# greatscottgadgets/libbtbb

Hardware: AMD Instinct MI355X
Metric: Gbit/s raw bitstream scanned (LAP_ANY, err<=2) (higher is better)
Workload: dtype u64; 1 GPU; promiscuous LAP_ANY scan, 4 GiB packed single-channel synthetic bitstream per GPU, max_ac_errors=2, sync word every 4096 symbols; symbols_per_gpu=34359738305, hits_per_gpu=6402406, parallelism=time-sharded x1 (btbbx_shard_plan: slices + 63-symbol halo), no collectives

## Files before the change

### libbtbb_amd/csrc/context.cpp

```cpp
#include <stdarg.h>
#include <stdio.h>
#include <stdlib.h>
#include <string.h>
#include <mutex>
#include <shared_mutex>
#include <vector>
#include "common.h"

#define NO_DEVICE_SLOT BTBBX_MAX_DEVICES
static Ctx g_ctx[BTBBX_MAX_DEVICES + 1];
static std::mutex g_init_lock;
static std::shared_mutex g_tables_lock;

void ctx_scan_snapshot(ScanTables *tables, int *table_errors)
{
	std::shared_lock<std::shared_mutex> g(g_tables_lock);
	const Ctx &c = ctx();
	*tables = c.scan;
	*table_errors = c.table_errors;
}
static int g_table_errors = 0;
static thread_local char g_err[512] = "";

static int current_device()
// ... 527 lines not shown
	return BTBBX_OK;
}

static int init_current_device(int max_ac_errors)
{
	const int dev = current_device();
	if (dev == NO_DEVICE_SLOT) {
		int d = -1;
		(void)hipGetDevice(&d);
		set_error("btbbx_init: HIP device ordinal %d is not below BTBBX_MAX_DEVICES = %d (or hipGetDevice failed)", d,
			  BTBBX_MAX_DEVICES);
		return BTBBX_E_ARG;
	}
	Ctx &c = g_ctx[dev];
	if (g_table_errors == 0 && max_ac_errors > 0)
		g_table_errors = max_ac_errors;
	if (!c.ready) {
		int n = 0;
		hipError_t e = hipGetDeviceCount(&n);
		if (e != hipSuccess || n <= 0) {
			set_error("btbbx_init: no HIP device available (%s) -- this library has no CPU path",
				  e == hipSuccess ? "device count 0" : hipGetErrorString(e));
			return BTBBX_E_NODEVICE;
		}
		c.device = dev;
		hipDeviceProp_t prop;
		HIP_TRY(hipGetDeviceProperties(&prop, dev));
		c.num_cus = prop.multiProcessorCount > 0 ? prop.multiProcessorCount : 256;
		int rc = chain_upload(host_tables());
		if (rc)
			return rc;
		rc = upload_tables(g_table_errors);
		if (rc)
			return rc;
		c.ready = true;
		return BTBBX_OK;
	}
	if (c.table_errors != g_table_errors)
		return upload_tables(g_table_errors);
	return BTBBX_OK;
}

extern "C" int btbbx_init(int max_ac_errors)
{
	if (max_ac_errors < 0 || max_ac_errors > 5) {
		set_error("btbbx_init: max_ac_errors out of range");
		return BTBBX_E_ARG;
	}
	std::lock_guard<std::mutex> g(g_init_lock);
	return init_current_device(max_ac_errors);
}

extern "C" int btbbx_init_devices(const int *devices, int n_devices, int max_ac_errors)
{
	if (max_ac_errors < 0 || max_ac_errors > 5 || n_devices < 0 || (n_devices && !devices)) {
		set_error("btbbx_init_devices: bad argument");
		return BTBBX_E_ARG;
	}
	const int have = btbbx_device_count();
	int home = 0;
	if (have <= 0 || hipGetDevice(&home) != hipSuccess) {
		set_error("btbbx_init_devices: no HIP device available -- this library has no CPU path");
		return BTBBX_E_NODEVICE;
	}
	std::lock_guard<std::mutex> g(g_init_lock);
	int rc = BTBBX_OK;
	for (int i = 0; i < n_devices && !rc; i++) {
		if (devices[i] < 0 || devices[i] >= have || devices[i] >= BTBBX_MAX_DEVICES) {
			set_error("btbbx_init_devices: device %d does not exist (%d visible)", devices[i], have);
			rc = BTBBX_E_ARG;
			break;
		}
		if (hipSetDevice(devices[i]) != hipSuccess)
			rc = hip_fail(hipGetLastError(), "hipSetDevice");
		else
			rc = init_current_device(max_ac_errors);
	}
	(void)hipSetDevice(home);
	return rc;
}

void hop_pool_release();
void sort_scratch_release();

extern "C" void btbbx_shutdown(void)
{
	std::lock_guard<std::mutex> g(g_init_lock);
	int home = 0;
	(void)hipGetDevice(&home);
	hop_pool_release();
	sort_scratch_release();
	for (int d = 0; d < BTBBX_MAX_DEVICES; d++) {
		Ctx &c = g_ctx[d];
		std::vector<CallBufs *> mine;
		{
			std::lock_guard<std::mutex> p(g_pool_lock);
			mine.swap(g_pool[d]);
		}
		if (!c.ready && mine.empty())
			continue;
		(void)hipSetDevice(d);
		for (CallBufs *b : mine)
			bufs_free(b);
		if (c.d_tab_block) (void)hipFree(c.d_tab_block);
		if (c.d_hslots) (void)hipFree(c.d_hslots);
		if (c.d_bitmap2) (void)hipFree(c.d_bitmap2);
		if (c.d_retired_tab) (void)hipFree(c.d_retired_tab);
		if (c.d_retired_hslots) (void)hipFree(c.d_retired_hslots);
		if (c.d_retired_bitmap2) (void)hipFree(c.d_retired_bitmap2);
		c = Ctx();
	}
	g_table_errors = 0;
	(void)hipSetDevice(home);
}


extern "C" void *btbbx_malloc(size_t bytes)
{
	void *p = nullptr;
	hipError_t e = hipMalloc(&p, bytes);
	if (e != hipSuccess) {
		hip_fail(e, "hipMalloc");
		return nullptr;
	}
	return p;
}

extern "C" void btbbx_free(void *p)
{
	if (p)
		(void)hipFree(p);
}

extern "C" int btbbx_memcpy_h2d(void *dst, const void *src, size_t bytes)
{
	HIP_TRY(hipMemcpy(dst, src, bytes, hipMemcpyHostToDevice));
	return BTBBX_OK;
}

extern "C" int btbbx_memcpy_d2h(void *dst, const void *src, size_t bytes)
{
	HIP_TRY(hipMemcpy(dst, src, bytes, hipMemcpyDeviceToHost));
	return BTBBX_OK;
}

extern "C" int btbbx_memset(void *p, int value, size_t bytes)
{
	HIP_TRY(hipMemset(p, value, bytes));
	return BTBBX_OK;
}

extern "C" int btbbx_sync(void *hip_stream)
{
	HIP_TRY(hipStreamSynchronize((hipStream_t)hip_stream));
	return BTBBX_OK;
}
```

### libbtbb_amd/csrc/packet.hip

```cpp
#include <stdlib.h>
#include <string.h>
#include <atomic>
#include <type_traits>
#include "packet_launch.h"
#include "packet_core.h"

static uint32_t host_crc_byte(uint32_t crc, uint32_t byte)
{
	uint32_t x = (crc ^ byte) & 0xff;
	x ^= (x << 4) & 0xff;
	return ((crc >> 8) ^ (x << 8) ^ (x << 3) ^ (x >> 4)) & 0xffff;
}

int chain_upload(const HostTables &t)
{
	{
		int seen[16] = {0};
		for (int clk = 0; clk < 64; clk++) {
			uint32_t v = 0;
			for (int j = 0; j < 4; j++)
				v |= (uint32_t)t.whiten[(t.whiten_idx[clk] + 3 + j) % 127] << j;
			seen[v]++;
		}
		for (int v = 0; v < 16; v++)
			if (seen[v] != 4) {
				set_error("btbbx_init: internal: the type-field whitening is not four clocks per value");
				return BTBBX_E_ARG;
			}
	}
	{
		static ChainLds img;
		memset(&img, 0, sizeof(img));
		for (int i = 0; i < 128; i++)
			for (int j = 0; j < 32; j++)
				img.wh32[i] |= (uint32_t)t.whiten[((i < 127 ? i : 0) + j) % 127] << j;
		for (int i = 0; i < 256; i++) {
			uint32_t c = host_crc_byte(0, (uint32_t)i);
			img.crc[i] = (uint16_t)c;
			for (int k = 0; k < 3; k++) {
				c = host_crc_byte(c, 0);
				img.crc_z[k][i] = (uint16_t)c;
			}
		}
		for (int i = 0; i < 1024; i++) {
			uint32_t par = 0;
			for (int bit = 0; bit < 10; bit++)
				if ((i >> bit) & 1)
					par ^= t.fec23_par[bit];
			img.par23[i] = (uint8_t)par;
		}
		memcpy(img.fix23, t.fec23_fix, 32);
		for (int i = 0; i < 32; i++)
			img.fixm23[i] = t.fec23_fix[i] == -2 ? 0x8000u : t.fec23_fix[i] >= 0 ? (uint16_t)(1u << t.fec23_fix[i]) : 0u;
		memcpy(img.whiten_idx, t.whiten_idx, 64);
		for (int h = 0; h < 2; h++)
			for (int i = 0; i < 256; i++) {
				uint32_t c = (uint32_t)i << (8 * h);
				for (int k = 0; k < 32; k++)
					c = host_crc_byte(c, 0);
				img.adv32[h][i] = (uint16_t)c;
			}
		HIP_TRY(hipMemcpyToSymbol(HIP_SYMBOL(g_chain_lds_image), &img, sizeof(img)));
	}
	{
		static uint16_t lin[LIN_MAXLEN * 16];
		memset(lin, 0, sizeof(lin));
		for (int bit = 0; bit < 8; bit++) {
			uint32_t crc = 1u << (8 + bit);
			for (int L = 0; L < LIN_MAXLEN; L++) {
				lin[L * 16 + bit] = (uint16_t)crc;
				crc = host_crc_byte(crc, 0);
			}
		}
		uint32_t taps = 0;
		for (uint32_t m = 1; m < 128 && !taps; m++) {
			bool ok = true;
			for (int k = 0; k < 127 && ok; k++) {
				uint32_t x = 0;
				for (int j = 0; j < 7; j++)
					if ((m >> j) & 1)
						x ^= t.whiten[(k + j) % 127];
				ok = x == t.whiten[(k + 7) % 127];
			}
			if (ok)
				taps = m;
// ... 94 lines not shown
	if (d_count)
		n_packets = min(n_packets, *d_count);
	uint32_t pkt = blockIdx.x * GATHER_PACKETS + threadIdx.x / BTBBX_PKT_WORDS;
	uint32_t i = threadIdx.x % BTBBX_PKT_WORDS;
	if (pkt >= n_packets || threadIdx.x >= GATHER_PACKETS * BTBBX_PKT_WORDS)
		return;
	const btbbx_hit h = hits[pkt];
	const uint64_t *base = words + (uint64_t)h.stream * pitch_words;
	uint64_t total_bits = n_words * 64;
	uint64_t avail = h.offset < total_bits ? total_bits - h.offset : 0;
	uint32_t len = avail < max_length ? (uint32_t)avail : max_length;
	if (len > BTBBX_MAX_SYMBOLS)
		len = BTBBX_MAX_SYMBOLS;
	uint64_t bit = h.offset + 64ULL * i;
	uint64_t j = bit >> 6;
	uint32_t sh = (uint32_t)(bit & 63);
	uint64_t lo = j < n_words ? base[j] : 0, hi = (j + 1) < n_words ? base[j + 1] : 0;
	uint64_t v = sh ? (lo >> sh) | (hi << (64 - sh)) : lo;
	uint32_t first = 64 * i;
	if (first >= len)
		v = 0;
	else if (len - first < 64)
		v &= (1ULL << (len - first)) - 1;
	packets[(uint64_t)pkt * BTBBX_PKT_WORDS + i] = v;
	if (i == 0)
		lengths[pkt] = len;
}

__global__ __launch_bounds__(256) void header_flags_kernel(const uint64_t *packets, const uint32_t *lengths, uint32_t n_packets,
							    uint8_t *present, const uint32_t *d_count)
{
	const uint32_t i = blockIdx.x * 256 + threadIdx.x;
	if (i >= n_packets || (d_count && i >= *d_count))
		return;
	PState s;
	s.w = packets + (uint64_t)i * BTBBX_PKT_WORDS;
	s.length = (int)lengths[i];
	present[i] = (uint8_t)do_header_present(s);
}

int launch_trials_state(const uint8_t *d_sym, const btbbx_pkt_in *d_in, const btbbx_pkt_out *d_out, void *d_state,
			btbbx_trial *d_trials, hipStream_t stream)
{
	int rc = ctx_require();
	if (rc)
		return rc;
	hipLaunchKernelGGL(trials_state_kernel, dim3(64), dim3(64), 0, stream, d_sym, d_in, d_out, (TrialState *)d_state, d_trials);
	HIP_TRY(hipGetLastError());
	return BTBBX_OK;
}

int launch_trials_merge(const void *d_state, const btbbx_pkt_in *d_in, btbbx_pkt_out *d_out, uint8_t *d_pay,
			const TrialPlan *plan, hipStream_t stream)
{
	hipLaunchKernelGGL(trials_merge_kernel, dim3(1), dim3(64), 0, stream, (const TrialState *)d_state, d_in, d_out, d_pay,
			   *plan);
	HIP_TRY(hipGetLastError());
	return BTBBX_OK;
}

size_t trials_state_bytes() { return 64 * sizeof(TrialState); }

int launch_gather(const uint64_t *d_words, uint64_t n_words, uint64_t pitch_words, const btbbx_hit *d_hits, uint32_t n_packets,
		  const uint32_t *d_count, uint32_t max_length, uint64_t *d_packets, uint32_t *d_lengths, hipStream_t hip_stream)
{
	int rc = ctx_require();
	if (rc)
		return rc;
	if (!n_packets)
		return BTBBX_OK;
	hipLaunchKernelGGL(gather_kernel, dim3((n_packets + GATHER_PACKETS - 1) / GATHER_PACKETS), dim3(256), 0,
			   hip_stream, d_words, n_words, pitch_words, d_hits, n_packets, max_length, d_packets, d_lengths, d_count);
	HIP_TRY(hipGetLastError());
	return BTBBX_OK;
}

extern "C" int btbbx_gather_packets_device(const uint64_t *d_words, uint64_t n_words, uint64_t pitch_words,
					   const btbbx_hit *d_hits, uint32_t n_packets, uint32_t max_length,
					   uint64_t *d_packets, uint32_t *d_lengths, void *hip_stream)
{
	return launch_gather(d_words, n_words, pitch_words, d_hits, n_packets, nullptr, max_length, d_packets, d_lengths, (hipStream_t)hip_stream);
}

extern "C" int btbbx_trials_device(const uint64_t *d_packets, const btbbx_pkt_in *d_in, uint32_t n_packets,
				   btbbx_trial *d_trials, void *hip_stream)
{
	return launch_trials(d_packets, d_in, n_packets, nullptr, d_trials, (hipStream_t)hip_stream);
}

int launch_trials(const uint64_t *d_packets, const btbbx_pkt_in *d_in, uint32_t n_packets, const uint32_t *d_count,
		  btbbx_trial *d_trials, hipStream_t hip_stream)
{
	int rc = ctx_require();
	if (rc)
		return rc;
	if (!n_packets)
		return BTBBX_OK;
	if (n_packets <= 256) {
		hipLaunchKernelGGL(trials_wide_kernel, dim3(n_packets * 64), dim3(64), 0, (hipStream_t)hip_stream,
				   d_packets, d_in, n_packets, d_trials, d_count);
	} else {
		const uint32_t batches = (n_packets + TL_PACKETS - 1) / TL_PACKETS;
		const uint32_t resident = (uint32_t)ctx().num_cus * TL_WGS_PER_CU;
		hipLaunchKernelGGL(trials_linear_kernel, dim3(batches < resident ? batches : resident), dim3(TL_THREADS), 0,
				   (hipStream_t)hip_stream, d_packets, d_in, n_packets, d_trials, d_count);
	}
#ifdef TL_PROFILE
	if (n_packets > 256) {
		unsigned long long prof[16], tot = 0;
		(void)hipDeviceSynchronize();
		(void)hipMemcpyFromSymbol(prof, HIP_SYMBOL(g_tl_prof), sizeof(prof));
		for (int k = 0; k < 16; k++) tot += prof[k];
		fprintf(stderr, "trials profile:");
		for (int k = 0; k < 10; k++) fprintf(stderr, " %d:%.1f%%", k, 100.0 * (double)prof[k] / (double)(tot ? tot : 1));
		fprintf(stderr, "\n");
		static unsigned long long z[16];
		(void)hipMemcpyToSymbol(HIP_SYMBOL(g_tl_prof), z, sizeof(z));
	}
#endif
	HIP_TRY(hipGetLastError());
	return BTBBX_OK;
}

extern "C" int btbbx_uap_table_device(const uint64_t *d_packets, const btbbx_pkt_in *d_in, uint32_t n_packets,
				      uint16_t *d_table, void *hip_stream)
{
	int rc = ctx_require();
	if (rc)
		return rc;
	if (!n_packets)
		return BTBBX_OK;
	if ((uintptr_t)d_table & 15) {
		set_error("btbbx_uap_table_device: table must be 16-byte aligned");
		return BTBBX_E_ARG;
	}
	hipLaunchKernelGGL(uap_table_kernel, dim3((n_packets + 255) / 256), dim3(256), 0, (hipStream_t)hip_stream,
			   d_packets, d_in, n_packets, (uint4 *)d_table);
	HIP_TRY(hipGetLastError());
	return BTBBX_OK;
}

int launch_header_flags(const uint64_t *d_packets, const uint32_t *d_lengths, uint32_t n_packets, const uint32_t *d_count,
			uint8_t *d_present, hipStream_t stream)
{
	if (!n_packets)
		return BTBBX_OK;
	hipLaunchKernelGGL(header_flags_kernel, dim3((n_packets + 255) / 256), dim3(256), 0, stream, d_packets, d_lengths, n_packets, d_present, d_count);
	HIP_TRY(hipGetLastError());
	return BTBBX_OK;
}

int launch_decode_bytes(const uint8_t *d_sym, uint8_t *d_pay, const btbbx_pkt_in *d_in, btbbx_pkt_out *d_out,
			uint32_t mode, bool with_payload, hipStream_t stream)
{
	int rc = ctx_require();
	if (rc)
		return rc;
	hipLaunchKernelGGL(decode_bytes_kernel, dim3(1), dim3(64), 0, stream, d_sym, d_pay, d_in, d_out, mode,
			   with_payload ? 1 : 0);
	HIP_TRY(hipGetLastError());
	return BTBBX_OK;
}

int launch_decode(const uint64_t *d_packets, const btbbx_pkt_in *d_in, uint32_t n_packets,
		  btbbx_pkt_out *d_out, uint32_t mode, const TrialPlan *plan, hipStream_t stream)
{
	int rc = ctx_require();
	if (rc)
		return rc;
	if (!n_packets)
		return BTBBX_OK;
	TrialPlan p = {0, 0, 0};
	if (plan)
		p = *plan;
	if (mode & DEC_TRIALS) {
		if (mode != DEC_TRIALS || n_packets != 1) {
			set_error("decode: trial replay is a one-packet mode");
			return BTBBX_E_ARG;
		}
		hipLaunchKernelGGL(replay_kernel, dim3(1), dim3(64), 0, stream, d_packets, d_in, d_out, p);
		HIP_TRY(hipGetLastError());
		return BTBBX_OK;
	}
	hipLaunchKernelGGL(decode_kernel, dim3((n_packets + 63) / 64), dim3(64), 0, stream,
			   d_packets, d_in, n_packets, d_out, mode);
	HIP_TRY(hipGetLastError());
	return BTBBX_OK;
}

extern "C" int btbbx_decode_device(const uint64_t *d_packets, const btbbx_pkt_in *d_in, uint32_t n_packets,
// ... 134 lines not shown
```

### libbtbb_amd/csrc/packet_trials.h

```cpp
#pragma once


__device__ __forceinline__ uint32_t lds_now(const uint32_t *p)
{
	return *(volatile __attribute__((address_space(3))) const uint32_t *)p;
}

#define TL_THREADS 512
#define TL_PACKETS (TL_THREADS / 16)
#define TL_WGS_PER_CU (1024 / TL_THREADS)
#define TL_TRIALS  (TL_PACKETS * 64)
#define TL_A_BLOCKS 183
#define TL_A_BYTES  232
#define TL_B_BLOCKS 10
#define TL_B_BYTES  16
#ifdef TL_PROFILE
__device__ unsigned long long g_tl_prof[16];
#define TL_PROF_START __shared__ uint32_t tl_acc[16]; if (threadIdx.x < 16) tl_acc[threadIdx.x] = 0; uint64_t tl_t = __builtin_readcyclecounter()
#define TL_PROF(k) do { const uint64_t n_ = __builtin_readcyclecounter(); if (tid == 0) tl_acc[k] += (uint32_t)(n_ - tl_t); tl_t = n_; } while (0)
#define TL_PROF_END do { __syncthreads(); if (tid < 16) atomicAdd(&g_tl_prof[tid], (unsigned long long)tl_acc[tid]); } while (0)
#else
#define TL_PROF_START do { } while (0)
#define TL_PROF(k) do { } while (0)
#define TL_PROF_END do { } while (0)
// ... 348 lines not shown
				if (hit) rv = 1000;
			}
			break;
		}
		case 3: case 8: case 10: case 14:
		case 4: case 11: case 15: {
			const bool fec = type == 3 || type == 8 || type == 10 || type == 14;
			const int layout = !fec ? 0 : (type == 8 ? 2 : 1);
			const int psize = type == 8 ? size - 80 : size;
			const int hb = (type == 3 || type == 8 || type == 4) ? 1 : 2;
			const int hbits = 8 * hb;
			const uint32_t fail = layout == 2 ? b_fail[p] : a_fail[p];
			rv = 0;
			if (psize < hbits) break;
			uint32_t raw;
			if (fec) {
				if (psize < (hb == 2 ? 30 : 15)) break;
				if (fail < (uint32_t)hb) break;
				raw = (layout == 2 ? b_bytes[p][0] : a_bytes[p][0]) & ((1u << hbits) - 1);
			} else {
				raw = pk_bits32(pk[p], 122, hbits);
			}
			const uint32_t ph = raw ^ (wht ? (uint32_t)wh_bits(wh_start(clock, 18), hbits) : 0u);
			int plen = hb == 2 ? (int)((ph >> 3) & 0x3ff) + 4 : (int)((ph >> 3) & 0x1f) + 3;
			int cap;
			switch (type) {
			case 3:  cap = 20;  break;
			case 4:  cap = 30;  break;
			case 8:  cap = 12;  break;
			case 10: cap = 125; break;
			case 11: cap = 187; break;
			case 14: cap = 228; break;
			default: cap = 343; break;
			}
			if (plen > cap) plen = cap;
			const int nbits = plen * 8;
			if (nbits > psize) { rv = 1; break; }
			if (fec && fail < (uint32_t)(nbits + 9) / 10) break;
			rv = crc_is_zero(layout, (uint32_t)plen) ? 10 : 2;
			break;
		}
		case 12: {
			uint32_t B = size >= 15 ? (uint32_t)size / 15 : 0;
			if (B > 98) B = 98;
			if (B > a_fail[p]) B = a_fail[p];
			const uint32_t lmax = B ? 5 * (B - 1) / 4 : 0;
			uint32_t crc = seed, idx = wh_start(clock, 18);
			rv = B == 98 ? 2 : 1;
			for (uint32_t L0 = 0; L0 < lmax; L0 += 4) {
				const uint32_t w = a_bytes[p][L0 >> 2] ^ (wht ? (uint32_t)wh_bits(idx, 32) : 0u);
				idx = idx + 32 >= 127 ? idx + 32 - 127 : idx + 32;
				const uint32_t x0 = (crc ^ w) & 0xff, x1 = ((crc ^ w) >> 8) & 0xff, b2 = (w >> 16) & 0xff, b3 = w >> 24;
				const uint32_t c1 = (crc >> 8) ^ g_lds.crc[x0];
				const uint32_t c2 = g_lds.crc_z[0][x0] ^ g_lds.crc[x1];
				const uint32_t c3 = g_lds.crc_z[1][x0] ^ g_lds.crc_z[0][x1] ^ g_lds.crc[b2];
				const uint32_t c4 = g_lds.crc_z[2][x0] ^ g_lds.crc_z[1][x1] ^ g_lds.crc_z[0][b2] ^ g_lds.crc[b3];
				const bool z1 = c1 == 0 && L0 + 1 >= 2 && L0 + 1 <= lmax, z2 = c2 == 0 && L0 + 2 <= lmax;
				const bool z3 = c3 == 0 && L0 + 3 <= lmax, z4 = c4 == 0 && L0 + 4 <= lmax;
				if (z1 || z2 || z3 || z4) { rv = 10; break; }
				crc = c4;
			}
			break;
		}
		case 5: rv = hv_rv[p]; break;
		default: rv = 1; break;
		}
		if (rv == 0 && type != 2 && type != 3 && type != 5)
			rv = 1;
		t_rv[i] = (int16_t)rv;
	}
	__syncthreads();
	TL_PROF(5);
	stage_in(batch + gridDim.x);
	fetch(batch + 2 * gridDim.x);
	static_assert(sizeof(btbbx_trial) == 4, "one dword per trial");
	for (uint32_t i = tid; i < total; i += TL_THREADS)
		reinterpret_cast<uint32_t *>(trials)[(uint64_t)first * 64 + i] =
			(t_info[i] & 0xffff) | ((uint32_t)(uint16_t)t_rv[i] << 16);
	TL_PROF(6);
	}
	TL_PROF_END;
}

__global__ __launch_bounds__(64) void trials_wide_kernel(const uint64_t *packets, const btbbx_pkt_in *in,
							  uint32_t n_packets, btbbx_trial *trials, const uint32_t *d_count)
{
	chain_lds_init();
	if (d_count)
		n_packets = min(n_packets, *d_count);
	const uint32_t pkt = blockIdx.x >> 6, clock = blockIdx.x & 63;
	if (threadIdx.x || pkt >= n_packets)
		return;
	const btbbx_pkt_in pi = in[pkt];
	PState s;
	s.w = packets + (uint64_t)pkt * BTBBX_PKT_WORDS;
	s.length = (int)pi.length;
	pstate_enter(s, pi);
	pstate_blank_out(s);
	uint32_t dis;
	const uint32_t hdr = header_fec13(s.w, dis);
	const uint32_t uap = do_try_clock(s, clock, hdr, dis);
	const int rv = do_crc_check<false>(s, clock);
	btbbx_trial t;
	t.uap = (uint8_t)uap;
	t.type = (uint8_t)s.type;
	t.rv = (int16_t)rv;
	trials[(uint64_t)pkt * 64 + clock] = t;
}

__global__ __launch_bounds__(256) void uap_table_kernel(const uint64_t *packets, const btbbx_pkt_in *in, uint32_t n,
							 uint4 *table)
{
	const uint32_t lane = threadIdx.x & 63;
	const uint32_t pkt0 = (blockIdx.x * 4 + (threadIdx.x >> 6)) * 64;
	if (pkt0 >= n)
		return;
	uint32_t ut = 0;
	if (pkt0 + lane < n) {
		const uint32_t p = pkt0 + lane;
		uint32_t dis;
		const uint32_t hdr = fec13((packets[(uint64_t)p * BTBBX_PKT_WORDS + 1] >> 4) & ((1ULL << 54) - 1), 18, dis);
		const uint32_t wht = in ? (in[p].flags & F_WHITENED) : 1u;
		ut = uap_from_hec(hdr & 0x3ff, hdr >> 10) | (((hdr >> 3) & 0xf) << 8) | ((dis < 4 ? 1u : 0u) << 16) | (wht << 17);
	}
	uint32_t wc[4] = {0, 0, 0, 0};
#pragma unroll
	for (int k = 0; k < 8; k++) {
		const uint32_t wb = (uint32_t)wh_bits_const(wh_start_const(8 * (lane & 7) + k, 0), 18);
		const uint32_t e = uap_from_hec(wb & 0x3ff, wb >> 10) | (((wb >> 3) & 0xf) << 8);
		wc[k >> 1] |= e << (16 * (k & 1));
	}
#pragma unroll
	for (int j = 0; j < 8; j++) {
		const uint32_t src = 8 * j + (lane >> 3);
		const uint32_t v = (uint32_t)__shfl((int)ut, (int)src);
		const uint32_t both = (v & 0xffff) * 0x10001u;
		const uint32_t okm = 0u - ((v >> 16) & 1u), whm = 0u - ((v >> 17) & 1u);
		uint4 o;
		o.x = (both ^ (wc[0] & whm)) & okm;
		o.y = (both ^ (wc[1] & whm)) & okm;
		o.z = (both ^ (wc[2] & whm)) & okm;
		o.w = (both ^ (wc[3] & whm)) & okm;
		if (pkt0 + src < n)
			table[(uint64_t)(pkt0 + src) * 8 + (lane & 7)] = o;
	}
}
```

Baseline: 12810 Gbit/s.

## Split fused trials kernel into prepare and run kernels via per-stream record buffer

Replaces the single fused trials_linear_kernel with two kernels. A prepare kernel decodes the FEC blocks, computes CRC chunk states and header data into a 40-row per-packet record in global memory. A run kernel then loads those records and evaluates the 64 clock trials per packet. Work is processed in chunks sized to whole resident passes, each kernel gets its own block size and occupancy tuning, and a per-stream scratch buffer is allocated lazily and freed at shutdown. The cost is an extra global round trip for the records and an extra launch per chunk. The fused path stays available behind a compile flag.

```diff
diff --git a/libbtbb_amd/csrc/context.cpp b/libbtbb_amd/csrc/context.cpp
--- a/libbtbb_amd/csrc/context.cpp
+++ b/libbtbb_amd/csrc/context.cpp
@@ -633,6 +633,7 @@
 
 void hop_pool_release();
 void sort_scratch_release();
+void trials_records_release();
 
 extern "C" void btbbx_shutdown(void)
 {
@@ -641,6 +642,7 @@
 	(void)hipGetDevice(&home);
 	hop_pool_release();
 	sort_scratch_release();
+	trials_records_release();
 	for (int d = 0; d < BTBBX_MAX_DEVICES; d++) {
 		Ctx &c = g_ctx[d];
 		std::vector<CallBufs *> mine;
diff --git a/libbtbb_amd/csrc/packet.hip b/libbtbb_amd/csrc/packet.hip
--- a/libbtbb_amd/csrc/packet.hip
+++ b/libbtbb_amd/csrc/packet.hip
@@ -1,6 +1,9 @@
 #include <stdlib.h>
 #include <string.h>
 #include <atomic>
+#include <mutex>
+#include <utility>
+#include <vector>
 #include <type_traits>
 #include "packet_launch.h"
 #include "packet_core.h"
@@ -261,6 +264,64 @@
 	return launch_gather(d_words, n_words, pitch_words, d_hits, n_packets, nullptr, max_length, d_packets, d_lengths, (hipStream_t)hip_stream);
 }
 
+static uint32_t trials_chunk_capacity(uint32_t cus) { return cus * (TP_WGS_PER_CU * TP_PACKETS) * 4u; }
+static_assert(TP_WGS_PER_CU * TP_PACKETS == TT_WGS_PER_CU * TT_PACKETS, "a chunk is whole passes of both grids");
+static uint32_t trials_chunk_packets(uint32_t cus)
+{
+	const uint32_t cap = trials_chunk_capacity(cus);
+	const char *e = getenv("BTBBX_TRIALS_CHUNK");
+	if (e && *e) {
+		const unsigned long v = strtoul(e, nullptr, 10);
+		if (v >= 1 && v < cap)
+			return (uint32_t)v;
+	}
+	return cap;
+}
+
+struct TrialRecords {
+	std::mutex lock;
+	std::vector<std::pair<hipStream_t, void *>> blocks;
+};
+static TrialRecords trial_records[BTBBX_MAX_DEVICES];
+
+static int trials_records(hipStream_t stream, size_t bytes, uint4 **block)
+{
+	int dev = 0;
+	if (hipGetDevice(&dev) != hipSuccess || dev < 0 || dev >= BTBBX_MAX_DEVICES) {
+		set_error("btbbx_trials_device: HIP device ordinal outside the %d contexts this library keeps", BTBBX_MAX_DEVICES);
+		return BTBBX_E_ARG;
+	}
+	TrialRecords &t = trial_records[dev];
+	std::lock_guard<std::mutex> g(t.lock);
+	for (const auto &b : t.blocks)
+		if (b.first == stream) {
+			*block = (uint4 *)b.second;
+			return BTBBX_OK;
+		}
+	void *p = nullptr;
+	HIP_TRY(hipMalloc(&p, bytes));
+	t.blocks.emplace_back(stream, p);
+	*block = (uint4 *)p;
+	return BTBBX_OK;
+}
+
+void trials_records_release()
+{
+	int home = 0;
+	(void)hipGetDevice(&home);
+	for (int d = 0; d < BTBBX_MAX_DEVICES; d++) {
+		TrialRecords &t = trial_records[d];
+		std::lock_guard<std::mutex> g(t.lock);
+		if (t.blocks.empty())
+			continue;
+		(void)hipSetDevice(d);
+		for (const auto &b : t.blocks)
+			(void)hipFree(b.second);
+		t.blocks.clear();
+	}
+	(void)hipSetDevice(home);
+}
+
 extern "C" int btbbx_trials_device(const uint64_t *d_packets, const btbbx_pkt_in *d_in, uint32_t n_packets,
 				   btbbx_trial *d_trials, void *hip_stream)
 {
@@ -279,12 +340,30 @@
 		hipLaunchKernelGGL(trials_wide_kernel, dim3(n_packets * 64), dim3(64), 0, (hipStream_t)hip_stream,
 				   d_packets, d_in, n_packets, d_trials, d_count);
 	} else {
+#ifdef BTBBX_TRIALS_FUSED
 		const uint32_t batches = (n_packets + TL_PACKETS - 1) / TL_PACKETS;
 		const uint32_t resident = (uint32_t)ctx().num_cus * TL_WGS_PER_CU;
 		hipLaunchKernelGGL(trials_linear_kernel, dim3(batches < resident ? batches : resident), dim3(TL_THREADS), 0,
 				   (hipStream_t)hip_stream, d_packets, d_in, n_packets, d_trials, d_count);
-	}
-#ifdef TL_PROFILE
+#else
+		const uint32_t cus = (uint32_t)ctx().num_cus;
+		const uint32_t chunk = trials_chunk_packets(cus);
+		uint4 *records = nullptr;
+		rc = trials_records(hip_stream, (size_t)trials_chunk_capacity(cus) * TR_ROWS * sizeof(uint4), &records);
+		if (rc)
+			return rc;
+		for (uint32_t at = 0; at < n_packets; at += chunk) {
+			const uint32_t cap = n_packets - at < chunk ? n_packets - at : chunk;
+			const uint32_t bp = (cap + TP_PACKETS - 1) / TP_PACKETS, bt = (cap + TT_PACKETS - 1) / TT_PACKETS;
+			const uint64_t *pk = d_packets + (uint64_t)at * BTBBX_PKT_WORDS;
+			hipLaunchKernelGGL(trials_prepare_kernel, dim3(bp < cus * TP_WGS_PER_CU ? bp : cus * TP_WGS_PER_CU), dim3(TP_THREADS), 0,
+					   hip_stream, pk, d_in + at, cap, at, records, d_count);
+			hipLaunchKernelGGL(trials_run_kernel, dim3(bt < cus * TT_WGS_PER_CU ? bt : cus * TT_WGS_PER_CU), dim3(TT_THREADS), 0,
+					   hip_stream, records, pk, cap, at, d_trials + (uint64_t)at * 64, d_count);
+		}
+#endif
+	}
+#if defined(TL_PROFILE) && defined(BTBBX_TRIALS_FUSED)
 	if (n_packets > 256) {
 		unsigned long long prof[16], tot = 0;
 		(void)hipDeviceSynchronize();
diff --git a/libbtbb_amd/csrc/packet_trials.h b/libbtbb_amd/csrc/packet_trials.h
--- a/libbtbb_amd/csrc/packet_trials.h
+++ b/libbtbb_amd/csrc/packet_trials.h
@@ -454,6 +454,523 @@
 	TL_PROF_END;
 }
 
+#define TR_PIN  0
+#define TR_HDR  1
+#define TR_BB   2
+#define TR_P4B  3
+#define TR_AB   6
+#define TR_P4A  21
+#define TR_P4C  29
+#define TR_ROWS 40
+#define TR_LDS_ROWS (TR_ROWS + 1)
+static_assert(16 * (TR_AB - TR_P4B) >= 8 + 2 * 20 && 16 * (TR_P4A - TR_AB) >= TL_A_BYTES && 16 * (TR_P4C - TR_P4A) >= 2 * (TL_A_BYTES / 4) &&
+	      16 * (TR_ROWS - TR_P4C) >= 2 * (LIN_MAXLEN / 4) && TL_B_BYTES == 16, "the parts of a record lie in their rows");
+
+#define TP_THREADS 512
+#define TP_PACKETS (TP_THREADS / 16)
+#define TP_WGS_PER_CU 3
+#define TT_THREADS 768
+#define TT_PACKETS (TT_THREADS / 16)
+#define TT_WGS_PER_CU 2
+#define TT_TRIALS  (TT_PACKETS * 64)
+
+__global__ __launch_bounds__(TP_THREADS) __attribute__((amdgpu_waves_per_eu(6, 6))) void trials_prepare_kernel(const uint64_t *packets, const btbbx_pkt_in *in,
+							      uint32_t n_packets, uint32_t list_first, uint4 *records, const uint32_t *d_count)
+{
+	if (d_count) {
+		const uint32_t n = *d_count;
+		n_packets = min(n_packets, n > list_first ? n - list_first : 0u);
+	}
+	__shared__ uint64_t pk[TP_PACKETS][BTBBX_PKT_WORDS + 1];
+	__shared__ __attribute__((aligned(16))) btbbx_pkt_in pin[TP_PACKETS];
+	__shared__ uint4 rec[TP_PACKETS][TR_LDS_ROWS];
+	__shared__ uint32_t hdr_ut[TP_PACKETS], hv_raw[TP_PACKETS];
+	__shared__ uint16_t a10[TP_PACKETS][TL_A_BLOCKS + 3];
+	__shared__ uint16_t b10[TP_PACKETS][TL_B_BLOCKS + 2];
+	__shared__ uint32_t a_fail[TP_PACKETS], b_fail[TP_PACKETS];
+	auto a_bytes = [&](uint32_t p) { return reinterpret_cast<uint32_t *>(&rec[p][TR_AB]); };
+	auto b_bytes = [&](uint32_t p) { return reinterpret_cast<uint32_t *>(&rec[p][TR_BB]); };
+	auto p4a = [&](uint32_t p) { return reinterpret_cast<uint16_t *>(&rec[p][TR_P4A]); };
+	auto p4b = [&](uint32_t p) { return reinterpret_cast<uint16_t *>(&rec[p][TR_P4B]); };
+	auto p4c = [&](uint32_t p) { return reinterpret_cast<uint16_t *>(&rec[p][TR_P4C]); };
+	auto chunk_reg = [&](uint32_t p) { return reinterpret_cast<uint16_t *>(&rec[p][TR_P4B]) + 4; };
+	const uint32_t tid = threadIdx.x;
+	chain_lds_init();
+	const uint32_t n_batches = (n_packets + TP_PACKETS - 1) / TP_PACKETS;
+	constexpr uint32_t PK_ELEMS = TP_PACKETS * (BTBBX_PKT_WORDS + 1), IN_ELEMS = TP_PACKETS * sizeof(btbbx_pkt_in) / 8;
+	constexpr uint32_t PER_THREAD = (PK_ELEMS + IN_ELEMS + TP_THREADS - 1) / TP_THREADS;
+	static_assert(sizeof(btbbx_pkt_in) == 16, "two words per btbbx_pkt_in");
+	uint64_t pre[PER_THREAD];
+	auto fetch = [&](uint32_t b) {
+		const uint32_t f = b * TP_PACKETS, have = b < n_batches ? (n_packets - f < TP_PACKETS ? n_packets - f : TP_PACKETS) : 0;
+		uint32_t tv = tid;
+		asm volatile("" : "+v"(tv));
+#pragma unroll
+		for (uint32_t k = 0; k < PER_THREAD; k++) {
+			const uint32_t i = tv + TP_THREADS * k;
+			const uint32_t p = i / (BTBBX_PKT_WORDS + 1), w = i % (BTBBX_PKT_WORDS + 1), e = i - PK_ELEMS;
+			const uint64_t *src = packets;
+			if (i < PK_ELEMS) {
+				if (p < have && w < BTBBX_PKT_WORDS)
+					src = packets + (uint64_t)(f + p) * BTBBX_PKT_WORDS + w;
+			} else if (e < 2 * have) {
+				src = reinterpret_cast<const uint64_t *>(in) + (uint64_t)f * 2 + e;
+			}
+			pre[k] = *src;
+		}
+	};
+	auto stage_in = [&](uint32_t b) {
+		const uint32_t f = b * TP_PACKETS, have = b < n_batches ? (n_packets - f < TP_PACKETS ? n_packets - f : TP_PACKETS) : 0;
+		uint32_t tv = tid;
+		asm volatile("" : "+v"(tv));
+#pragma unroll
+		for (uint32_t k = 0; k < PER_THREAD; k++) {
+			const uint32_t i = tv + TP_THREADS * k;
+			const uint32_t p = i / (BTBBX_PKT_WORDS + 1), w = i % (BTBBX_PKT_WORDS + 1);
+			if (i < PK_ELEMS)
+				pk[p][w] = (p < have && w < BTBBX_PKT_WORDS) ? pre[k] : 0;
+			else if (i < PK_ELEMS + IN_ELEMS)
+				reinterpret_cast<uint64_t *>(pin)[i - PK_ELEMS] = pre[k];
+		}
+		if (tid < TP_PACKETS) {
+			a_fail[tid] = TL_A_BLOCKS;
+			b_fail[tid] = TL_B_BLOCKS;
+		}
+	};
+	fetch(blockIdx.x);
+	stage_in(blockIdx.x);
+	fetch(blockIdx.x + gridDim.x);
+	for (uint32_t batch = blockIdx.x; batch < n_batches; batch += gridDim.x) {
+	const uint32_t first = batch * TP_PACKETS;
+	const uint32_t mine = n_packets - first < TP_PACKETS ? n_packets - first : TP_PACKETS;
+
+	__syncthreads();
+
+	if (tid < mine) {
+		uint32_t dis;
+		const uint32_t hdr = header_fec13(pk[tid], dis);
+		hdr_ut[tid] = uap_from_hec(hdr & 0x3ff, hdr >> 10) | (((hdr >> 3) & 0xf) << 8) | ((dis < 4 ? 1u : 0u) << 16);
+	}
+	static_assert(TP_THREADS == 16 * TP_PACKETS, "sixteen threads per packet");
+	auto a_words = [&](uint32_t p) {
+		const uint32_t blocks = TL_AFAIL(p) < TL_A_BLOCKS ? TL_AFAIL(p) : TL_A_BLOCKS, n = (blocks * 10 + 31) / 32 + 1;
+		return n < TL_A_BYTES / 4 ? n : (uint32_t)(TL_A_BYTES / 4);
+	};
+	{
+		const uint32_t p = tid >> 4, sub = tid & 15;
+		if (p < mine) {
+			uint32_t d;
+			if (sub < TL_B_BLOCKS) {
+				if (!fec23_block(pk_bits32(pk[p], 202 + 15 * sub, 15), d))
+					atomicMin(&b_fail[p], sub);
+				b10[p][sub] = (uint16_t)d;
+			}
+#pragma unroll 1
+			for (uint32_t k0 = 0; k0 < TL_A_BLOCKS; k0 += 16) {
+				const uint32_t k = k0 + sub;
+				if (k < TL_A_BLOCKS) {
+					if (!fec23_block(pk_bits32(pk[p], 122 + 15 * k, 15), d))
+						atomicMin(&a_fail[p], k);
+					a10[p][k] = (uint16_t)d;
+				}
+				__builtin_amdgcn_fence(__ATOMIC_ACQ_REL, "wavefront");
+				if (TL_AFAIL(p) < k0 + 16)
+					break;
+			}
+			__builtin_amdgcn_fence(__ATOMIC_ACQ_REL, "wavefront");
+			auto word_from = [&](const uint16_t *src, uint32_t nblk, uint32_t word) {
+				const uint32_t bit = 32 * word, k0 = bit / 10, sh = bit % 10;
+				uint64_t acc = 0;
+				for (uint32_t j = 0; j < 5; j++)
+					acc |= (uint64_t)(k0 + j < nblk ? src[k0 + j] : 0) << (10 * j);
+				return (uint32_t)(acc >> sh);
+			};
+			if (sub < TL_B_BYTES / 4)
+				b_bytes(p)[sub] = word_from(b10[p], TL_B_BLOCKS, sub);
+			const uint32_t need = a_words(p);
+			for (uint32_t word = sub; word < need; word += 16)
+				a_bytes(p)[word] = word_from(a10[p], TL_A_BLOCKS, word);
+		}
+	}
+	if (tid >= 128 && tid < 128 + mine) {
+		const uint32_t p = tid - 128;
+		uint32_t rv = 1;
+		if ((int)pin[p].length - 122 >= 240) {
+			uint32_t total = 0;
+			for (int i = 0; i < 4; i++) {
+				uint32_t dis;
+				(void)fec13(pk_bits(pk[p], 122 + 60 * i, 60), 20, dis);
+				total += dis;
+			}
+			rv = total < 20 ? 2 : 0;
+		}
+		hv_raw[p] = rv | (pk_bits32(pk[p], 122, 16) << 16);
+	}
+	__syncthreads();
+	auto chunk_of = [&](uint32_t t, uint32_t &p, uint32_t &r, uint32_t &layout, uint32_t &j, uint32_t &nwords) {
+		if (t < mine * 12) {
+			p = t / 12;
+			j = t % 12;
+			if (j < 11) { layout = 0; r = j; nwords = j < 10 ? 8 : LIN_MAXLEN / 4 - 80; }
+			else { layout = 2; r = 19; j = 0; nwords = TL_B_BYTES / 4; }
+		} else {
+			const uint32_t u = t - mine * 12;
+			j = mine == TP_PACKETS ? u / TP_PACKETS : u / mine;
+			p = u - j * mine;
+			layout = 1;
+			r = 11 + j;
+			const uint32_t need = a_words(p);
+			nwords = need > 8 * j ? (need - 8 * j < 8 ? need - 8 * j : 8) : 0;
+		}
+	};
+	auto chunk_words = [&](uint32_t p, uint32_t layout, uint32_t j, uint32_t nwords, uint32_t (&w8)[8]) {
+		if (layout == 0) {
+			const uint32_t *d = reinterpret_cast<const uint32_t *>(pk[p]) + 3 + 8 * j;
+			uint32_t raw[9];
+#pragma unroll
+			for (uint32_t i = 0; i < 9; i++)
+				raw[i] = i <= nwords ? d[i] : 0;
+#pragma unroll
+			for (uint32_t i = 0; i < 8; i++)
+				w8[i] = __builtin_amdgcn_alignbit(raw[i + 1], raw[i], 26);
+		} else {
+			const uint32_t *src = layout == 1 ? a_bytes(p) : b_bytes(p);
+#pragma unroll
+			for (uint32_t i = 0; i < 8; i++)
+				w8[i] = i < nwords ? src[8 * j + i] : 0;
+		}
+	};
+	for (uint32_t t = tid; t < mine * 20; t += TP_THREADS) {
+		uint32_t p, r, layout, j, nwords, crc = 0;
+		chunk_of(t, p, r, layout, j, nwords);
+		if (!nwords)
+			continue;
+		uint32_t w8[8];
+		chunk_words(p, layout, j, nwords, w8);
+		uint16_t *dst = layout == 0 ? p4c(p) : layout == 1 ? p4a(p) : p4b(p);
+#pragma unroll
+		for (uint32_t i = 0; i < 8; i++)
+			if (i < nwords) {
+				dst[8 * j + i] = (uint16_t)crc;
+				crc = crc_word(crc, w8[i]);
+			}
+		chunk_reg(p)[r] = (uint16_t)crc;
+	}
+	__syncthreads();
+	if (tid < mine) {
+		rec[tid][TR_PIN] = *reinterpret_cast<const uint4 *>(&pin[tid]);
+		rec[tid][TR_HDR] = make_uint4(hdr_ut[tid], a_fail[tid], b_fail[tid], hv_raw[tid]);
+	}
+	if (tid >= 64 && tid < 64 + 3 * mine) {
+		const uint32_t p = (tid - 64) / 3, layout = (tid - 64) % 3;
+		const uint32_t r0 = layout == 0 ? 0 : layout == 1 ? 11 : 19;
+		const uint32_t n = layout == 0 ? 11 : layout == 1 ? (a_words(p) + 7) / 8 : 1;
+		uint32_t start = 0;
+		for (uint32_t j = 0; j < n; j++) {
+			const uint32_t c = chunk_reg(p)[r0 + j];
+			chunk_reg(p)[r0 + j] = (uint16_t)start;
+			start = g_lds.adv32[0][start & 0xff] ^ g_lds.adv32[1][start >> 8] ^ c;
+		}
+	}
+	__syncthreads();
+	stage_in(batch + gridDim.x);
+	fetch(batch + 2 * gridDim.x);
+	for (uint32_t i = tid; i < mine * TR_ROWS; i += TP_THREADS) {
+		const uint32_t p = i / TR_ROWS, r = i - p * TR_ROWS;
+		records[(uint64_t)first * TR_ROWS + i] = rec[p][r];
+	}
+	}
+}
+
+__global__ __launch_bounds__(TT_THREADS) __attribute__((amdgpu_waves_per_eu(6, 6))) void trials_run_kernel(const uint4 *records, const uint64_t *packets,
+							  uint32_t n_packets, uint32_t list_first, btbbx_trial *trials, const uint32_t *d_count)
+{
+	if (d_count) {
+		const uint32_t n = *d_count;
+		n_packets = min(n_packets, n > list_first ? n - list_first : 0u);
+	}
+	__shared__ uint4 rec[TT_PACKETS][TR_LDS_ROWS];
+	__shared__ uint16_t clk_ut[64];
+	__shared__ __attribute__((aligned(16))) uint16_t pw20[64];
+	__shared__ __attribute__((aligned(16))) uint16_t lin[LIN_MAXLEN * 16];
+	__shared__ __attribute__((aligned(16))) uint16_t advw[7 * 2 * 256];
+	__shared__ uint16_t order[TT_TRIALS];
+	__shared__ uint32_t t_info[TT_TRIALS];
+	__shared__ int16_t t_rv[TT_TRIALS];
+	__shared__ uint32_t pk_sort[TT_PACKETS];
+	__shared__ uint32_t type_base[18];
+	auto pin = [&](uint32_t p) -> const btbbx_pkt_in & { return *reinterpret_cast<const btbbx_pkt_in *>(&rec[p][TR_PIN]); };
+	auto hdr_row = [&](uint32_t p) { return reinterpret_cast<const uint32_t *>(&rec[p][TR_HDR]); };
+	auto a_bytes = [&](uint32_t p) { return reinterpret_cast<const uint32_t *>(&rec[p][TR_AB]); };
+	auto b_bytes = [&](uint32_t p) { return reinterpret_cast<const uint32_t *>(&rec[p][TR_BB]); };
+	auto p4a = [&](uint32_t p) { return reinterpret_cast<const uint16_t *>(&rec[p][TR_P4A]); };
+	auto p4b = [&](uint32_t p) { return reinterpret_cast<const uint16_t *>(&rec[p][TR_P4B]); };
+	auto p4c = [&](uint32_t p) { return reinterpret_cast<const uint16_t *>(&rec[p][TR_P4C]); };
+	auto chunk_reg = [&](uint32_t p) { return reinterpret_cast<const uint16_t *>(&rec[p][TR_P4B]) + 4; };
+	const uint32_t tid = threadIdx.x, lane = tid & 63;
+	for (uint32_t i = tid; i < LIN_MAXLEN * 2; i += TT_THREADS)
+		reinterpret_cast<uint4 *>(lin)[i] = reinterpret_cast<const uint4 *>(g_lin)[i];
+	for (uint32_t i = tid; i < 7 * 2 * 256 / 8; i += TT_THREADS)
+		reinterpret_cast<uint4 *>(advw)[i] = reinterpret_cast<const uint4 *>(g_advw)[i];
+	chain_lds_init();
+	if (tid >= 64 && tid < 128) {
+		const uint32_t wb = (uint32_t)wh_bits(wh_start(tid - 64, 0), 18);
+		const uint32_t wt = (wb >> 3) & 0xf;
+		uint32_t crank = 0;
+		for (uint32_t k = 0; k < 16; k++) {
+			const uint64_t mk = __ballot(wt == k);
+			if (wt == k)
+				crank = __builtin_amdgcn_mbcnt_hi((uint32_t)(mk >> 32), __builtin_amdgcn_mbcnt_lo((uint32_t)mk, 0));
+		}
+		clk_ut[tid - 64] = (uint16_t)(uap_from_hec(wb & 0x3ff, wb >> 10) | (wt << 8) | (crank << 12));
+		const uint32_t v = (uint32_t)wh_bits(wh_start(tid - 64, 18), 7);
+		uint32_t x = 0;
+		for (int j = 0; j < 7; j++)
+			if ((v >> j) & 1)
+				x ^= lin[20 * 16 + 8 + j];
+		pw20[tid - 64] = (uint16_t)x;
+	}
+	const uint32_t n_batches = (n_packets + TT_PACKETS - 1) / TT_PACKETS;
+	constexpr uint32_t REC_ELEMS = TT_PACKETS * TR_ROWS;
+	constexpr uint32_t PER_THREAD = (REC_ELEMS + TT_THREADS - 1) / TT_THREADS;
+	typedef uint32_t row_t __attribute__((ext_vector_type(4)));
+	row_t pre[PER_THREAD];
+	auto fetch = [&](uint32_t b) {
+		const uint32_t f = b * TT_PACKETS, have = b < n_batches ? (n_packets - f < TT_PACKETS ? n_packets - f : TT_PACKETS) : 0;
+		uint32_t tv = tid;
+		asm volatile("" : "+v"(tv));
+#pragma unroll
+		for (uint32_t k = 0; k < PER_THREAD; k++) {
+			const uint32_t i = tv + TT_THREADS * k;
+			const uint4 *src = records;
+			if (i < have * TR_ROWS)
+				src = records + (uint64_t)f * TR_ROWS + i;
+			pre[k] = *reinterpret_cast<const row_t *>(src);
+		}
+	};
+	auto stage_in = [&](uint32_t) {
+		uint32_t tv = tid;
+		asm volatile("" : "+v"(tv));
+#pragma unroll
+		for (uint32_t k = 0; k < PER_THREAD; k++) {
+			const uint32_t i = tv + TT_THREADS * k, p = i / TR_ROWS;
+			if (i < REC_ELEMS)
+				*reinterpret_cast<row_t *>(&rec[p][i - p * TR_ROWS]) = pre[k];
+		}
+	};
+	fetch(blockIdx.x);
+	stage_in(blockIdx.x);
+	fetch(blockIdx.x + gridDim.x);
+	for (uint32_t batch = blockIdx.x; batch < n_batches; batch += gridDim.x) {
+	const uint32_t first = batch * TT_PACKETS;
+	const uint32_t mine = n_packets - first < TT_PACKETS ? n_packets - first : TT_PACKETS;
+
+	__syncthreads();
+
+	static_assert(TT_PACKETS <= 64, "one wave ranks the packets of a batch");
+	if (tid < 64) {
+		const bool live = tid < mine;
+		const uint32_t h = live ? hdr_row(tid)[0] : 0u;
+		const bool fec_ok = (h & 0x10000u) != 0;
+		const bool var = live && fec_ok && (pin(live ? tid : 0).flags & F_WHITENED);
+		const uint32_t key = !live ? 0u : fec_ok ? (h >> 8) & 0xfu : (uint32_t)pin(tid).type & 0xfu;
+		const uint64_t vm = __ballot(var);
+		const uint32_t nvar = (uint32_t)__popcll(vm);
+		uint32_t rank = __builtin_amdgcn_mbcnt_hi((uint32_t)(vm >> 32), __builtin_amdgcn_mbcnt_lo((uint32_t)vm, 0));
+		const bool fixed = live && !var;
+		uint32_t cf = 0;
+		if (__ballot(fixed)) {
+			for (uint32_t k = 0; k < 16; k++) {
+				const uint64_t fm = __ballot(fixed && key == k);
+				if (fixed && key == k)
+					rank = __builtin_amdgcn_mbcnt_hi((uint32_t)(fm >> 32), __builtin_amdgcn_mbcnt_lo((uint32_t)fm, 0));
+				if (lane == k)
+					cf = (uint32_t)__popcll(fm);
+			}
+		}
+		uint32_t incl = cf;
+#pragma unroll
+		for (int dd = 1; dd < 16; dd <<= 1) {
+			const uint32_t up = __shfl_up(incl, dd);
+			if (lane >= (uint32_t)dd)
+				incl += up;
+		}
+		if (lane < 16)
+			type_base[lane] = 4u * nvar * lane + 64u * (incl - cf);
+		if (lane == 17)
+			type_base[17] = nvar;
+		if (tid < TT_PACKETS)
+			pk_sort[tid] = key | ((var ? 1u : 0u) << 4) | (rank << 8);
+	}
+	__syncthreads();
+	const uint32_t total = mine * 64;
+	for (uint32_t i = tid; i < total; i += TT_THREADS) {
+		const uint32_t p = i >> 6;
+		const uint32_t h = hdr_row(p)[0];
+		uint32_t uap = pin(p).uap, type = pin(p).type, ret = 0;
+		const uint32_t ps = pk_sort[p], cu = clk_ut[lane];
+		if (h & 0x10000u) {
+			const uint32_t v = (h ^ ((pin(p).flags & F_WHITENED) ? (cu & 0xfffu) : 0u)) & 0xffff;
+			uap = ret = v & 0xff;
+			type = v >> 8;
+		}
+		t_info[i] = ret | (type << 8) | (uap << 16);
+		const uint32_t slot = (ps & 0x10u) ? type_base[type & 15] + 4u * (ps >> 8) + (cu >> 12)
+						   : type_base[type & 15] + 4u * type_base[17] + 64u * (ps >> 8) + lane;
+		order[slot] = (uint16_t)i;
+	}
+	__syncthreads();
+
+	for (uint32_t kk = tid; kk < total; kk += TT_THREADS) {
+		const uint32_t i = order[kk], p = i >> 6, clock = i & 63;
+		const uint32_t info = t_info[i], type = (info >> 8) & 0xff, uap = (info >> 16) & 0xff;
+		const bool wht = pin(p).flags & F_WHITENED;
+		const int size = (int)pin(p).length - 122;
+		const uint32_t a_fail = hdr_row(p)[1], b_fail = hdr_row(p)[2];
+		const uint32_t seed = crc_seed(uap);
+		const uint32_t sel = (seed >> 8) | (wht ? (uint32_t)wh_bits(wh_start(clock, 18), 7) << 8 : 0u);
+		auto seed_row20 = [&](uint32_t sd) {
+			const uint4 r0 = reinterpret_cast<const uint4 *>(lin)[40];
+			const uint32_t r[4] = {r0.x, r0.y, r0.z, r0.w};
+			uint32_t x = 0;
+#pragma unroll
+			for (int bit = 0; bit < 8; bit++)
+				x ^= (0u - ((sd >> (8 + bit)) & 1)) & (r[bit >> 1] >> (16 * (bit & 1)));
+			return x & 0xffff;
+		};
+		auto lin_terms = [&](uint32_t L) {
+			uint32_t x = 0;
+#pragma unroll
+			for (int half = 0; half < 2; half++) {
+				const uint4 q = reinterpret_cast<const uint4 *>(lin)[2 * L + half];
+				const uint32_t r[4] = {q.x, q.y, q.z, q.w};
+				const uint32_t sl = sel >> (8 * half);
+#pragma unroll
+				for (int bit = 0; bit < 8; bit++)
+					x ^= (0u - ((sl >> bit) & 1)) & (r[bit >> 1] >> (16 * (bit & 1)));
+			}
+			return x & 0xffff;
+		};
+		auto data_reg = [&](int layout, uint32_t L) {
+			const uint32_t q = L >> 2, r = L & 3;
+			uint32_t crc, w = 0;
+			if (layout == 0) {
+				crc = p4c(p)[q];
+				if (r) {
+					const uint32_t *d = reinterpret_cast<const uint32_t *>(packets + (uint64_t)(first + p) * BTBBX_PKT_WORDS) + 3 + q;
+					w = __builtin_amdgcn_alignbit(d[1], d[0], 26);
+				}
+			}
+			else if (layout == 1) { crc = p4a(p)[q]; w = r ? a_bytes(p)[q] : 0; }
+			else { crc = p4b(p)[q]; w = r ? b_bytes(p)[q] : 0; }
+			const uint32_t start = chunk_reg(p)[(layout == 0 ? 0u : layout == 1 ? 11u : 19u) + (q >> 3)], iw = q & 7;
+			crc ^= iw ? (uint32_t)(advw[((iw - 1) * 2) * 256 + (start & 0xff)] ^ advw[((iw - 1) * 2 + 1) * 256 + (start >> 8)]) : start;
+			for (uint32_t j = 0; j < r; j++)
+				crc = crc_byte(crc, (w >> (8 * j)) & 0xff);
+			return crc;
+		};
+		auto crc_is_zero = [&](int layout, uint32_t L) {
+			return (data_reg(layout, L) ^ lin_terms(L)) == 0;
+		};
+		int rv = 1;
+		switch (type) {
+		case 2: {
+			if (size < 240) { rv = 1; break; }
+			if (a_fail < 16) { rv = 0; break; }
+			const uint32_t x = data_reg(1, 20) ^ seed_row20(seed);
+			rv = 0;
+			if (!wht) {
+				if (x == 0) rv = 1000;
+			} else {
+				uint32_t hit = x == pw20[clock];
+				const uint32_t xx = x | (x << 16);
+#pragma unroll 1
+				for (int v = 0; v < 4; v++) {
+					const uint4 q = reinterpret_cast<const uint4 *>(&pw20[32])[v];
+					const uint32_t d0 = q.x ^ xx, d1 = q.y ^ xx, d2 = q.z ^ xx, d3 = q.w ^ xx;
+					hit |= ((d0 & 0xffff) == 0) | ((d0 >> 16) == 0) | ((d1 & 0xffff) == 0) | ((d1 >> 16) == 0)
+					     | ((d2 & 0xffff) == 0) | ((d2 >> 16) == 0) | ((d3 & 0xffff) == 0) | ((d3 >> 16) == 0);
+				}
+				if (hit) rv = 1000;
+			}
+			break;
+		}
+		case 3: case 8: case 10: case 14:
+		case 4: case 11: case 15: {
+			const bool fec = type == 3 || type == 8 || type == 10 || type == 14;
+			const int layout = !fec ? 0 : (type == 8 ? 2 : 1);
+			const int psize = type == 8 ? size - 80 : size;
+			const int hb = (type == 3 || type == 8 || type == 4) ? 1 : 2;
+			const int hbits = 8 * hb;
+			const uint32_t fail = layout == 2 ? b_fail : a_fail;
+			rv = 0;
+			if (psize < hbits) break;
+			uint32_t raw;
+			if (fec) {
+				if (psize < (hb == 2 ? 30 : 15)) break;
+				if (fail < (uint32_t)hb) break;
+				raw = (layout == 2 ? b_bytes(p)[0] : a_bytes(p)[0]) & ((1u << hbits) - 1);
+			} else {
+				raw = (hdr_row(p)[3] >> 16) & ((1u << hbits) - 1);
+			}
+			const uint32_t ph = raw ^ (wht ? (uint32_t)wh_bits(wh_start(clock, 18), hbits) : 0u);
+			int plen = hb == 2 ? (int)((ph >> 3) & 0x3ff) + 4 : (int)((ph >> 3) & 0x1f) + 3;
+			int cap;
+			switch (type) {
+			case 3:  cap = 20;  break;
+			case 4:  cap = 30;  break;
+			case 8:  cap = 12;  break;
+			case 10: cap = 125; break;
+			case 11: cap = 187; break;
+			case 14: cap = 228; break;
+			default: cap = 343; break;
+			}
+			if (plen > cap) plen = cap;
+			const int nbits = plen * 8;
+			if (nbits > psize) { rv = 1; break; }
+			if (fec && fail < (uint32_t)(nbits + 9) / 10) break;
+			rv = crc_is_zero(layout, (uint32_t)plen) ? 10 : 2;
+			break;
+		}
+		case 12: {
+			uint32_t B = size >= 15 ? (uint32_t)size / 15 : 0;
+			if (B > 98) B = 98;
+			if (B > a_fail) B = a_fail;
+			const uint32_t lmax = B ? 5 * (B - 1) / 4 : 0;
+			uint32_t crc = seed, idx = wh_start(clock, 18);
+			rv = B == 98 ? 2 : 1;
+			for (uint32_t L0 = 0; L0 < lmax; L0 += 4) {
+				const uint32_t w = a_bytes(p)[L0 >> 2] ^ (wht ? (uint32_t)wh_bits(idx, 32) : 0u);
+				idx = idx + 32 >= 127 ? idx + 32 - 127 : idx + 32;
+				const uint32_t x0 = (crc ^ w) & 0xff, x1 = ((crc ^ w) >> 8) & 0xff, b2 = (w >> 16) & 0xff, b3 = w >> 24;
+				const uint32_t c1 = (crc >> 8) ^ g_lds.crc[x0];
+				const uint32_t c2 = g_lds.crc_z[0][x0] ^ g_lds.crc[x1];
+				const uint32_t c3 = g_lds.crc_z[1][x0] ^ g_lds.crc_z[0][x1] ^ g_lds.crc[b2];
+				const uint32_t c4 = g_lds.crc_z[2][x0] ^ g_lds.crc_z[1][x1] ^ g_lds.crc_z[0][b2] ^ g_lds.crc[b3];
+				const bool z1 = c1 == 0 && L0 + 1 >= 2 && L0 + 1 <= lmax, z2 = c2 == 0 && L0 + 2 <= lmax;
+				const bool z3 = c3 == 0 && L0 + 3 <= lmax, z4 = c4 == 0 && L0 + 4 <= lmax;
+				if (z1 || z2 || z3 || z4) { rv = 10; break; }
+				crc = c4;
+			}
+			break;
+		}
+		case 5: rv = (int)(int8_t)(hdr_row(p)[3] & 0xff); break;
+		default: rv = 1; break;
+		}
+		if (rv == 0 && type != 2 && type != 3 && type != 5)
+			rv = 1;
+		t_rv[i] = (int16_t)rv;
+	}
+	__syncthreads();
+	stage_in(batch + gridDim.x);
+	fetch(batch + 2 * gridDim.x);
+	static_assert(sizeof(btbbx_trial) == 4, "one dword per trial");
+	for (uint32_t i = tid; i < total; i += TT_THREADS)
+		reinterpret_cast<uint32_t *>(trials)[(uint64_t)first * 64 + i] =
+			(t_info[i] & 0xffff) | ((uint32_t)(uint16_t)t_rv[i] << 16);
+	}
+}
+
 __global__ __launch_bounds__(64) void trials_wide_kernel(const uint64_t *packets, const btbbx_pkt_in *in,
 							  uint32_t n_packets, btbbx_trial *trials, const uint32_t *d_count)
 {
```

Result: no change. 12830 Gbit/s (median of 5 runs) (+0.2%).
